# syun88/VLA-from-FastVLM

Measured on AMD Instinct MI355X. Metric: policy steps/sec (img+prompt->action) FastVLM-0.5B bs=64, higher is better.
Workload: dtype bf16; 1 GPU; fastvlm-0.5b select_action: letterbox 336^2->1024^2, FastViT-HD, projector, Qwen2 decoder (text-only, reference-literal: 64-token prompt), last-token pool, action head; batch_per_gpu=64, global_batch=64, seq_len=64, image=336, parallelism=replicas x1 (no collective on the inference path), tower_microbatch=0, stream_overlap=True, llm_precision=split-bf16 (hi+lo) operands, fp32 attention

## Files before the change

vla-from-fastvlm_amd/csrc/tower_kernels.hip:

```cpp
#include "kernels.h"
#include <cstdlib>

namespace fv {
namespace {

struct LbParams {
  const void* img; bf16_t* pix; int dtype, B, C, Hin, Win, S, rh, rw, pt, pl; float pad, sh, sw;
};

__device__ __forceinline__ float lb_fetch(const LbParams& p, size_t plane, int y, int x) {
  const size_t i = plane + (size_t)y * p.Win + x;
  return p.dtype == FV_U8 ? (float)static_cast<const uint8_t*>(p.img)[i] : static_cast<const float*>(p.img)[i];
}

__device__ __forceinline__ float lb_lerp(float a, float b, float w) {
#pragma clang fp contract(off)
  return (1.0f - w) * a + w * b;
}
__device__ __forceinline__ float lb_src(int d, float scale) {
#pragma clang fp contract(off)
  return fmaxf(((float)d + 0.5f) * scale - 0.5f, 0.0f);
}
__device__ __forceinline__ float lb_frac(float s, int i) {
#pragma clang fp contract(off)
// ... 497 lines not shown
        *reinterpret_cast<uint4*>(y + (((size_t)b * S2 + oy) * S2 + ox) * SF_C + cg * 8) = o;
      }
    }
    if (tile_n < (unsigned)ntiles) patch_store();
  }
}

typedef __attribute__((ext_vector_type(4))) short s16x4;

template <int K, int TH>
__global__ __launch_bounds__(256, TH == 8 ? 3 : 2) void dwconv_mfma_kernel(const bf16_t* __restrict__ x, const bf16_t* __restrict__ ttab,
                                                              const float* __restrict__ bias, bf16_t* __restrict__ y,
                                                              int H, int W, int C, int gelu, int tiles_x, int tiles_y,
                                                              int nslices) {
  constexpr int TW = 32, NP = TH / 8, PAD = K / 2, IH = TH + K - 1, IW = TW + K - 1;
  constexpr int NQ = (IW + 3) / 4, NM = (K + 3 + 3) / 4;
  constexpr int RS = NQ * 256 + 64;
  constexpr int T_BYTES = 2 * K * NM * 512, X_BYTES = IH * RS;
  __shared__ __attribute__((aligned(16))) char smem[X_BYTES];
  char* sX = smem;

  const int tid = threadIdx.x, lane = tid & 63, wid = tid >> 6;
#ifdef DW_NO_XCD
  int bid = blockIdx.x;
#else
  int bid = xcd_remap(blockIdx.x, gridDim.x);
#endif
  const int slice = bid % nslices; bid /= nslices;
  const int tx = bid % tiles_x; bid /= tiles_x;
  const int tyb = bid % tiles_y;
  const long b = bid / tiles_y;
  const int c0 = slice * 32;
  const int gg = wid & 1, rg = wid >> 1;
  const int bch = lane >> 2, jr = lane & 3;

  s16x4 afr[K][NM];
  {
    const char* tsrc = reinterpret_cast<const char*>(ttab) + (size_t)slice * T_BYTES + (size_t)gg * K * NM * 512 + lane * 8;
#pragma unroll
    for (int ky = 0; ky < K; ++ky)
#pragma unroll
      for (int m = 0; m < NM; ++m) afr[ky][m] = __builtin_bit_cast(s16x4, *reinterpret_cast<const uint2*>(tsrc + (ky * NM + m) * 512));
  }
  constexpr int NTASK = IH * NQ * 4, TPT = (NTASK + 255) / 256;
  uint4 px[TPT][4];
#pragma unroll
  for (int tt = 0; tt < TPT; ++tt) {
    const int task = tid + 256 * tt;
    const int cg = task & 3, quad = (task >> 2) % NQ, row = (task >> 2) / NQ;
    const int iy = tyb * TH - PAD + row, ix0 = tx * TW - PAD + quad * 4;
#pragma unroll
    for (int j = 0; j < 4; ++j) {
      const int ix = ix0 + j;
      px[tt][j] = (task < NTASK && iy >= 0 && iy < H && ix >= 0 && ix < W && quad * 4 + j < IW)
                      ? *reinterpret_cast<const uint4*>(x + (((size_t)b * H + iy) * W + ix) * C + c0 + cg * 8)
                      : make_uint4(0, 0, 0, 0);
    }
  }
#pragma unroll
  for (int tt = 0; tt < TPT; ++tt) {
    const int task = tid + 256 * tt;
    if (task < NTASK) {
      const int cg = task & 3, quad = (task >> 2) % NQ, row = (task >> 2) / NQ;
      const uint32_t d[4][4] = {{px[tt][0].x, px[tt][0].y, px[tt][0].z, px[tt][0].w}, {px[tt][1].x, px[tt][1].y, px[tt][1].z, px[tt][1].w},
                                {px[tt][2].x, px[tt][2].y, px[tt][2].z, px[tt][2].w}, {px[tt][3].x, px[tt][3].y, px[tt][3].z, px[tt][3].w}};
      const uint32_t dst = (uint32_t)(row * RS + quad * 256 + cg * 64) | (uint32_t)((((quad & 3) << 1) | (cg >> 1)) << 3);
#pragma unroll
      for (int dd = 0; dd < 4; ++dd) {
        uint2 ev, od;
        ev.x = __builtin_amdgcn_perm(d[1][dd], d[0][dd], 0x05040100u);
        ev.y = __builtin_amdgcn_perm(d[3][dd], d[2][dd], 0x05040100u);
        od.x = __builtin_amdgcn_perm(d[1][dd], d[0][dd], 0x07060302u);
        od.y = __builtin_amdgcn_perm(d[3][dd], d[2][dd], 0x07060302u);
        *reinterpret_cast<uint2*>(sX + (dst ^ (uint32_t)((2 * dd) * 8))) = ev;
        *reinterpret_cast<uint2*>(sX + (dst ^ (uint32_t)((2 * dd + 1) * 8))) = od;
      }
    }
  }
  __syncthreads();

  const char* lrow[4];
#pragma unroll
  for (int v = 0; v < 4; ++v) lrow[v] = sX + (rg * 4 * NP + jr) * RS + (((gg * 16 + bch) ^ ((v << 1) | gg)) << 3);
  f32x4 acc[NP][8];
#pragma unroll
  for (int pp = 0; pp < NP; ++pp)
#pragma unroll
    for (int q = 0; q < 8; ++q) acc[pp][q] = f32x4{0.f, 0.f, 0.f, 0.f};
#pragma unroll
  for (int pp = 0; pp < NP; ++pp)
#pragma unroll
    for (int ky = 0; ky < K; ++ky) {
      s16x4 xq[NQ];
#pragma unroll
      for (int t = 0; t < NQ; ++t)
        xq[t] = __builtin_bit_cast(s16x4, *reinterpret_cast<const uint2*>(lrow[t & 3] + (pp * 4 + ky) * RS + t * 256));
#pragma unroll
      for (int q = 0; q < 8; ++q)
#pragma unroll
        for (int m = 0; m < NM; ++m)
#ifdef DW_ABL_MFMA
          if (q + m < NQ && m == 0) acc[pp][q] = __builtin_amdgcn_mfma_f32_4x4x4bf16_1k(afr[ky][m], xq[q + m], acc[pp][q], 0, 0, 0);
#else
          if (q + m < NQ) acc[pp][q] = __builtin_amdgcn_mfma_f32_4x4x4bf16_1k(afr[ky][m], xq[q + m], acc[pp][q], 0, 0, 0);
#endif
    }
  __syncthreads();

  {
    const float bv = bias[c0 + gg * 16 + bch];
#pragma unroll
    for (int pp = 0; pp < NP; ++pp)
#pragma unroll
      for (int q = 0; q < 8; ++q) {
        float v[4];
#pragma unroll
        for (int i = 0; i < 4; ++i) {
          v[i] = acc[pp][q][i] + bv;
          if (gelu) v[i] = gelu_f(v[i]);
        }
        uint2 u;
        u.x = pack_bf2(v[0], v[1]);
        u.y = pack_bf2(v[2], v[3]);
        *reinterpret_cast<uint2*>(const_cast<char*>(lrow[q & 3]) + pp * 4 * RS + q * 256) = u;
      }
  }
  __syncthreads();
#pragma unroll
  for (int ot = 0; ot < NP; ++ot) {
    const int task = tid + 256 * ot;
    const int cg = task & 3, quad = (task >> 2) & 7, row = task >> 5;
    const uint32_t src = (uint32_t)(row * RS + quad * 256 + cg * 64) | (uint32_t)((((quad & 3) << 1) | (cg >> 1)) << 3);
    uint2 r[8];
#pragma unroll
    for (int e = 0; e < 8; ++e) r[e] = *reinterpret_cast<const uint2*>(sX + (src ^ (uint32_t)(e * 8)));
    const int oy = tyb * TH + row, ox0 = tx * TW + quad * 4;
    if (oy < H) {
      bf16_t* yp = y + (((size_t)b * H + oy) * W + ox0) * C + c0 + cg * 8;
#pragma unroll
      for (int j = 0; j < 4; ++j) {
        if (ox0 + j < W) {
          uint4 o;
          const uint32_t sel = (j & 1) ? 0x07060302u : 0x05040100u;
#define FV_PX(A, B) __builtin_amdgcn_perm((j & 2) ? r[B].y : r[B].x, (j & 2) ? r[A].y : r[A].x, sel)
          o.x = FV_PX(0, 1); o.y = FV_PX(2, 3); o.z = FV_PX(4, 5); o.w = FV_PX(6, 7);
#undef FV_PX
          *reinterpret_cast<uint4*>(yp + (size_t)j * C) = o;
        }
      }
    }
  }
}

__global__ __launch_bounds__(256, 2) void dwconv_s2_mfma_kernel(const bf16_t* __restrict__ x, const bf16_t* __restrict__ ttab,
                                                                 const float* __restrict__ bias, bf16_t* __restrict__ y, int H,
                                                                 int W, int C, int Ho, int Wo, int gelu, int tiles_x, int tiles_y,
                                                                 int nslices, int nimg) {
  constexpr int K = 7, TH = 8, TW = 16, PAD = 3, IH = 2 * TH + K - 2, IW = 2 * TW + K - 2;
  constexpr int NQ = (IW + 3) / 4, NM = 4;
  constexpr int RS = NQ * 256 + 64;
  constexpr int X_BYTES = IH * RS;
  constexpr int OC = 512 + 16;
  static_assert(TH * 4 * OC <= X_BYTES, "the output tile reuses the halo tile's LDS");
  __shared__ __attribute__((aligned(16))) char smem[X_BYTES];
  char* sX = smem;
  const int tid = threadIdx.x, lane = tid & 63, wid = tid >> 6;
  const int xcd = blockIdx.x & 7, lb = blockIdx.x >> 3;
  const int slice = lb % nslices, chain = lb / nslices, chains = (int)(gridDim.x >> 3) / nslices;
  const int ntiles = nimg * tiles_x * tiles_y;
  const int tpx = (ntiles + 7) >> 3, t_end = min((xcd + 1) * tpx, ntiles), per_slice = chains;
  const int c0 = slice * 32;
  const int gg = wid & 1, eo = wid >> 1;
  const int bch = lane >> 2, jr = lane & 3;

  s16x4 afr[K][NM];
  {
    const char* tsrc = reinterpret_cast<const char*>(ttab) + (size_t)(slice * 2 + gg) * (2 * K * NM * 512) + (size_t)eo * (K * NM * 512) + lane * 8;
#pragma unroll
    for (int ky = 0; ky < K; ++ky)
#pragma unroll
      for (int m = 0; m < NM; ++m) afr[ky][m] = __builtin_bit_cast(s16x4, *reinterpret_cast<const uint2*>(tsrc + (ky * NM + m) * 512));
  }
  constexpr int NTASK = IH * NQ * 4, TPT = (NTASK + 255) / 256;
  uint4 px[TPT][4];
  int trow[TPT], tcol[TPT], toff[TPT];
  uint32_t tdst[TPT];
#pragma unroll
  for (int tt = 0; tt < TPT; ++tt) {
    const int task = min(tid + 256 * tt, NTASK - 1);
    const int cg = task & 3, quad = (task >> 2) % NQ, row = (task >> 2) / NQ;
    trow[tt] = row;
    tcol[tt] = quad * 4;
    toff[tt] = (row * W + quad * 4) * C + cg * 8;
    tdst[tt] = (uint32_t)(row * RS + quad * 256 + cg * 64) | (uint32_t)((((quad & 3) << 1) | (cg >> 1)) << 3);
  }
  auto fetch = [&](int tx, int tyb, int b) {
    const int iy0 = 2 * tyb * TH - PAD, ix0 = 2 * tx * TW - PAD;
    const bf16_t* org = x + ((long)b * H * W + (long)iy0 * W + ix0) * C + c0;
#pragma unroll
    for (int tt = 0; tt < TPT; ++tt) {
      const bool rok = (unsigned)(iy0 + trow[tt]) < (unsigned)H;
#pragma unroll
      for (int j = 0; j < 4; ++j)
        px[tt][j] = (rok && (unsigned)(ix0 + tcol[tt] + j) < (unsigned)W) ? *reinterpret_cast<const uint4*>(org + toff[tt] + j * C)
                                                                         : make_uint4(0, 0, 0, 0);
    }
  };
  auto decode = [&](int tile, int& tx, int& tyb, int& b) {
    const unsigned t = (unsigned)tile, r = t / (unsigned)tiles_x;
    tx = (int)(t - r * (unsigned)tiles_x);
    b = (int)(r / (unsigned)tiles_y);
    tyb = (int)(r - (unsigned)b * (unsigned)tiles_y);
  };
  int tile = xcd * tpx + chain, tx = 0, tyb = 0, b = 0, txn = 0, tybn = 0, bn = 0;
  if (tile < t_end) { decode(tile, tx, tyb, b); fetch(tx, tyb, b); }
  for (; tile < t_end; tile += per_slice) {
#pragma unroll
  for (int tt = 0; tt < TPT; ++tt) {
    if (tid + 256 * tt < NTASK) {
      const uint32_t d[4][4] = {{px[tt][0].x, px[tt][0].y, px[tt][0].z, px[tt][0].w}, {px[tt][1].x, px[tt][1].y, px[tt][1].z, px[tt][1].w},
                                {px[tt][2].x, px[tt][2].y, px[tt][2].z, px[tt][2].w}, {px[tt][3].x, px[tt][3].y, px[tt][3].z, px[tt][3].w}};
      const uint32_t dst = tdst[tt];
#pragma unroll
      for (int dd = 0; dd < 4; ++dd) {
        uint2 ev, od;
        ev.x = __builtin_amdgcn_perm(d[1][dd], d[0][dd], 0x05040100u);
        ev.y = __builtin_amdgcn_perm(d[3][dd], d[2][dd], 0x05040100u);
        od.x = __builtin_amdgcn_perm(d[1][dd], d[0][dd], 0x07060302u);
        od.y = __builtin_amdgcn_perm(d[3][dd], d[2][dd], 0x07060302u);
        *reinterpret_cast<uint2*>(sX + (dst ^ (uint32_t)((2 * dd) * 8))) = ev;
        *reinterpret_cast<uint2*>(sX + (dst ^ (uint32_t)((2 * dd + 1) * 8))) = od;
      }
    }
  }
  __syncthreads();
  if (tile + per_slice < t_end) { decode(tile + per_slice, txn, tybn, bn); fetch(txn, tybn, bn); }

  const char* lrow[4];
#pragma unroll
  for (int v = 0; v < 4; ++v) lrow[v] = sX + (2 * jr) * RS + (((gg * 16 + bch) ^ ((v << 1) | gg)) << 3);
  f32x4 acc[2][4];
#pragma unroll
  for (int rg = 0; rg < 2; ++rg)
#pragma unroll
    for (int q = 0; q < 4; ++q) acc[rg][q] = f32x4{0.f, 0.f, 0.f, 0.f};
#pragma unroll
  for (int ky = 0; ky < K; ++ky)
#pragma unroll
    for (int rg = 0; rg < 2; ++rg) {
      s16x4 xq[NQ];
#pragma unroll
      for (int t = 0; t < NQ; ++t) xq[t] = __builtin_bit_cast(s16x4, *reinterpret_cast<const uint2*>(lrow[t & 3] + (rg * 8 + ky) * RS + t * 256));
#pragma unroll
      for (int m = 0; m < NM; ++m)
#pragma unroll
        for (int q = 0; q < 4; ++q) acc[rg][q] = __builtin_amdgcn_mfma_f32_4x4x4bf16_1k(afr[ky][m], xq[2 * q + m], acc[rg][q], 0, 0, 0);
    }
  __syncthreads();

  {
    const int co = 2 * (gg * 16 + bch) + eo, sig = (jr >> 1) & 1;
    const float bv = bias[2 * c0 + co];
#pragma unroll
    for (int rg = 0; rg < 2; ++rg)
#pragma unroll
      for (int q = 0; q < 4; ++q) {
        f32x2 g[2] = {{acc[rg][q][0] + bv, acc[rg][q][1] + bv}, {acc[rg][q][2] + bv, acc[rg][q][3] + bv}};
        if (gelu) gelu2_n<2>(g);
        uint2 u;
        u.x = pack_bf2(g[0].x, g[0].y);
        u.y = pack_bf2(g[1].x, g[1].y);
        *reinterpret_cast<uint2*>(sX + ((rg * 4 + jr) * 4 + q) * OC + ((co ^ sig) << 3)) = u;
      }
  }
  __syncthreads();
  {
    const int cg = tid & 7, quad = (tid >> 3) & 3, row = tid >> 5;
    const int sig = (row >> 1) & 1;
    uint2 r[8];
#pragma unroll
    for (int e = 0; e < 8; ++e) r[e] = *reinterpret_cast<const uint2*>(sX + (row * 4 + quad) * OC + (((cg * 8 + e) ^ sig) << 3));
    const int oy = tyb * TH + row, ox0 = tx * TW + quad * 4;
    if (oy < Ho) {
      bf16_t* yp = y + (((size_t)b * Ho + oy) * Wo + ox0) * (2 * C) + 2 * c0 + cg * 8;
#pragma unroll
      for (int j = 0; j < 4; ++j) {
        if (ox0 + j < Wo) {
          uint4 o;
          const uint32_t sel = (j & 1) ? 0x07060302u : 0x05040100u;
#define FV_PX(A, B) __builtin_amdgcn_perm((j & 2) ? r[B].y : r[B].x, (j & 2) ? r[A].y : r[A].x, sel)
          o.x = FV_PX(0, 1); o.y = FV_PX(2, 3); o.z = FV_PX(4, 5); o.w = FV_PX(6, 7);
#undef FV_PX
          *reinterpret_cast<uint4*>(yp + (size_t)j * (2 * C)) = o;
        }
      }
    }
  }
  __syncthreads();
  tx = txn; tyb = tybn; b = bn;
  }
}

#ifndef DW_MARCH_OCC
#define DW_MARCH_OCC 2
#endif
typedef __attribute__((ext_vector_type(4))) _Float16 f16x4_t;
template <int K, bool GRAD = false>
__global__ __launch_bounds__(256, DW_MARCH_OCC) void dwconv_march_kernel(const bf16_t* __restrict__ x, const bf16_t* __restrict__ ttab,
                                                               const float* __restrict__ bias, bf16_t* __restrict__ y,
                                                               int H, int W, int C, int gelu, int tiles_x, int nslices, const bf16_t* __restrict__ res = nullptr) {
  constexpr int TW = 32, PAD = K / 2, IW = TW + K - 1;
  constexpr int NQ = (IW + 3) / 4, NM = (K + 3 + 3) / 4;
  constexpr int RS = NQ * 256 + 64, RSO = 8 * 256 + 64;
  constexpr int T_BYTES = 2 * K * NM * 512;
#if DW_MARCH_OCC >= 3
  __shared__ __attribute__((aligned(16))) char smem[16 * RS];
#else
  __shared__ __attribute__((aligned(16))) char smem[16 * RS + 8 * RSO];
#endif
  char* sX = smem;

  const int tid = threadIdx.x, lane = tid & 63, wid = tid >> 6;
  int bid = xcd_remap(blockIdx.x, gridDim.x);
  const int slice = bid % nslices; bid /= nslices;
  const int tx = bid % tiles_x;
  const long b = bid / tiles_x;
  const int c0 = slice * 32;
  const int gg = wid & 1, rg = wid >> 1;
  const int bch = lane >> 2, jr = lane & 3;
  const int ng = (H + 7) / 8;

  s16x4 afr[K][NM];
  {
    const char* tsrc = reinterpret_cast<const char*>(ttab) + (size_t)slice * T_BYTES + (size_t)gg * K * NM * 512 + lane * 8;
#pragma unroll
    for (int ky = 0; ky < K; ++ky)
#pragma unroll
      for (int m = 0; m < NM; ++m) afr[ky][m] = __builtin_bit_cast(s16x4, *reinterpret_cast<const uint2*>(tsrc + (ky * NM + m) * 512));
  }
  const float bv = GRAD ? 0.f : bias[c0 + gg * 16 + bch];

  constexpr int NTASK = 8 * NQ * 4, TPT = (NTASK + 255) / 256;
  uint4 px[TPT][4];
#define DW_LOAD_UNIT(U)                                                                                          \
  {                                                                                                              \
    _Pragma("unroll") for (int tt = 0; tt < TPT; ++tt) {                                                         \
      const int task = tid + 256 * tt;                                                                           \
      const int cg = task & 3, quad = (task >> 2) % NQ, row = (task >> 2) / NQ;                                  \
      const int iy = 8 * (U) + PAD + row, ix0 = tx * TW - PAD + quad * 4;                                        \
      _Pragma("unroll") for (int j = 0; j < 4; ++j) {                                                            \
        const int ix = ix0 + j;                                                                                  \
        px[tt][j] = (task < NTASK && iy >= 0 && iy < H && ix >= 0 && ix < W && quad * 4 + j < IW)                \
                        ? *reinterpret_cast<const uint4*>(x + (((size_t)b * H + iy) * W + ix) * C + c0 + cg * 8)  \
                        : make_uint4(0, 0, 0, 0);                                                                \
      }                                                                                                          \
    }                                                                                                            \
  }
#define DW_WRITE_UNIT(U)                                                                                         \
  {                                                                                                              \
    _Pragma("unroll") for (int tt = 0; tt < TPT; ++tt) {                                                         \
      const int task = tid + 256 * tt;                                                                           \
      if (task < NTASK) {                                                                                        \
        const int cg = task & 3, quad = (task >> 2) % NQ, row = (task >> 2) / NQ;                                \
        const uint32_t d[4][4] = {{px[tt][0].x, px[tt][0].y, px[tt][0].z, px[tt][0].w},                          \
                                  {px[tt][1].x, px[tt][1].y, px[tt][1].z, px[tt][1].w},                          \
                                  {px[tt][2].x, px[tt][2].y, px[tt][2].z, px[tt][2].w},                          \
                                  {px[tt][3].x, px[tt][3].y, px[tt][3].z, px[tt][3].w}};                         \
        const uint32_t dst = (uint32_t)((8 * ((U) & 1) + row) * RS + quad * 256 + cg * 64) |                     \
                             (uint32_t)((((quad & 3) << 1) | (cg >> 1)) << 3);                                   \
        _Pragma("unroll") for (int dd = 0; dd < 4; ++dd) {                                                       \
          uint2 ev, od;                                                                                          \
          ev.x = __builtin_amdgcn_perm(d[1][dd], d[0][dd], 0x05040100u);                                         \
          ev.y = __builtin_amdgcn_perm(d[3][dd], d[2][dd], 0x05040100u);                                         \
          od.x = __builtin_amdgcn_perm(d[1][dd], d[0][dd], 0x07060302u);                                         \
          od.y = __builtin_amdgcn_perm(d[3][dd], d[2][dd], 0x07060302u);                                         \
          *reinterpret_cast<uint2*>(sX + (dst ^ (uint32_t)((2 * dd) * 8))) = ev;                                 \
          *reinterpret_cast<uint2*>(sX + (dst ^ (uint32_t)((2 * dd + 1) * 8))) = od;                             \
        }                                                                                                        \
      }                                                                                                          \
    }                                                                                                            \
  }
  uint32_t sw[4];
#pragma unroll
  for (int v = 0; v < 4; ++v) sw[v] = (uint32_t)(((gg * 16 + bch) ^ ((v << 1) | gg)) << 3);

  DW_LOAD_UNIT(-1)
  DW_WRITE_UNIT(-1)
  DW_LOAD_UNIT(0)
  DW_WRITE_UNIT(0)
  if (ng > 1) DW_LOAD_UNIT(1)

  for (int g = 0; g < ng; ++g) {
    __syncthreads();
    f32x4 acc[8];
#pragma unroll
    for (int q = 0; q < 8; ++q) acc[q] = f32x4{0.f, 0.f, 0.f, 0.f};
    const int rb = 8 * g + rg * 4 + jr - 2 * PAD;
#pragma unroll
    for (int ky = 0; ky < K; ++ky) {
      const uint32_t ro = (uint32_t)((rb + ky) & 15) * RS;
      s16x4 xq[NQ];
#pragma unroll
      for (int t = 0; t < NQ; ++t) xq[t] = __builtin_bit_cast(s16x4, *reinterpret_cast<const uint2*>(sX + ro + sw[t & 3] + t * 256));
#pragma unroll
      for (int m = 0; m < NM; ++m)
#pragma unroll
        for (int q = 0; q < 8; ++q)
          if (q + m < NQ) {
            if constexpr (GRAD) acc[q] = __builtin_amdgcn_mfma_f32_4x4x4f16(__builtin_bit_cast(f16x4_t, afr[ky][m]), __builtin_bit_cast(f16x4_t, xq[q + m]), acc[q], 0, 0, 0);
            else acc[q] = __builtin_amdgcn_mfma_f32_4x4x4bf16_1k(afr[ky][m], xq[q + m], acc[q], 0, 0, 0);
          }
    }
    __syncthreads();
#if DW_MARCH_OCC >= 3
    char* sO = sX + 8 * ((g + 1) & 1) * RS;
#else
    char* sO = smem + 16 * RS;
    if (g + 1 < ng) DW_WRITE_UNIT(g + 1)
    if (g + 2 < ng) DW_LOAD_UNIT(g + 2)
#endif
    {
      char* orow = sO + (rg * 4 + jr) * RSO;
#pragma unroll
      for (int q = 0; q < 8; ++q) {
        float v[4];
#pragma unroll
        for (int i = 0; i < 4; ++i) {
          v[i] = acc[q][i] + bv;
          if (gelu) v[i] = gelu_f(v[i]);
        }
        uint2 u;
        if constexpr (GRAD) { u.x = pack_h2(v[0], v[1]); u.y = pack_h2(v[2], v[3]); }
        else { u.x = pack_bf2(v[0], v[1]); u.y = pack_bf2(v[2], v[3]); }
        *reinterpret_cast<uint2*>(orow + sw[q & 3] + q * 256) = u;
      }
    }
    __syncthreads();
    {
      const int cg = tid & 3, quad = (tid >> 2) & 7, row = tid >> 5;
      const uint32_t src = (uint32_t)(row * RSO + quad * 256 + cg * 64) | (uint32_t)((((quad & 3) << 1) | (cg >> 1)) << 3);
      uint2 r[8];
#pragma unroll
      for (int e = 0; e < 8; ++e) r[e] = *reinterpret_cast<const uint2*>(sO + (src ^ (uint32_t)(e * 8)));
      const int oy = g * 8 + row, ox0 = tx * TW + quad * 4;
      if (oy < H) {
        bf16_t* yp = y + (((size_t)b * H + oy) * W + ox0) * C + c0 + cg * 8;
#pragma unroll
        for (int j = 0; j < 4; ++j) {
          if (ox0 + j < W) {
            uint4 o;
            const uint32_t sel = (j & 1) ? 0x07060302u : 0x05040100u;
#define FV_PX(A, B) __builtin_amdgcn_perm((j & 2) ? r[B].y : r[B].x, (j & 2) ? r[A].y : r[A].x, sel)
// ... 489 lines not shown
  p.img = img; p.pix = pix; p.dtype = dtype; p.B = B; p.C = C; p.Hin = Hin; p.Win = Win; p.S = S; p.pad = pad_value;
  if (letterbox) {
    const double ratio = ((double)Win / S > (double)Hin / S) ? (double)Win / S : (double)Hin / S;
    p.rh = (int)((double)Hin / ratio);
    p.rw = (int)((double)Win / ratio);
    if (p.rh > S || p.rw > S || p.rh < 1 || p.rw < 1) return fv_fail(FV_ERR_ARG, "letterbox: degenerate resize %dx%d", p.rh, p.rw);
  } else {
    p.rh = S; p.rw = S;
  }
  p.pt = S - p.rh; p.pl = S - p.rw;
  p.sh = (float)Hin / (float)p.rh;
  p.sw = (float)Win / (float)p.rw;
  return FV_OK;
}
}

int launch_letterbox(const void* img, int dtype, int B, int C, int Hin, int Win, int S, float pad_value, int letterbox,
                     bf16_t* pix, hipStream_t s) {
  if (!img || !pix) return fv_fail(FV_ERR_ARG, "letterbox: null pointer");
  LbParams p;
  FV_TRY_RC(lb_params(img, dtype, B, C, Hin, Win, S, pad_value, letterbox, pix, p));
  hipLaunchKernelGGL(letterbox_kernel<0>, dim3((S + 255) / 256, (S + LB_R - 1) / LB_R, B), dim3(256), 0, s, p, LbNorm{});
  FV_HIP_CHECK(hipGetLastError());
  return FV_OK;
}

int launch_letterbox_norm(const void* img, int dtype, int B, int C, int Hin, int Win, int S, float pad_value, int letterbox, const float* mean3,
                          const float* std3, int range_heuristic, unsigned* vmax_scratch, bf16_t* pix, hipStream_t s) {
  if (!img || !pix || !mean3 || !std3 || (range_heuristic && !vmax_scratch)) return fv_fail(FV_ERR_ARG, "letterbox_norm: null pointer");
  LbParams p;
  FV_TRY_RC(lb_params(img, dtype, B, C, Hin, Win, S, pad_value, letterbox, pix, p));
  LbNorm n{};
  for (int c = 0; c < 3; ++c) {
    if (!(std3[c] != 0.0f)) return fv_fail(FV_ERR_ARG, "letterbox_norm: std[%d] must be non-zero", c);
    n.mean[c] = mean3[c]; n.std[c] = std3[c];
  }
  n.vmax = vmax_scratch; n.heuristic = range_heuristic ? 1 : 0;
  const dim3 grid((S + 255) / 256, (S + LB_R - 1) / LB_R, B);
  if (range_heuristic) {
    FV_HIP_CHECK(hipMemsetAsync(vmax_scratch, 0, 4, s));
    hipLaunchKernelGGL(letterbox_kernel<1>, grid, dim3(256), 0, s, p, n);
  }
  hipLaunchKernelGGL(letterbox_kernel<2>, grid, dim3(256), 0, s, p, n);
  FV_HIP_CHECK(hipGetLastError());
  return FV_OK;
}

int launch_stem_conv(const bf16_t* pix, const float* w, const float* bias, bf16_t* y, int B, int S, int Cout,
                     hipStream_t s) {
  if (!pix || !w || !bias || !y) return fv_fail(FV_ERR_ARG, "stem_conv: null pointer");
  if (B <= 0 || S < 2 || (S & 1) || Cout % 8 || Cout < 8 || Cout > 2048) return fv_fail(FV_ERR_ARG, "stem_conv: bad shape S=%d Cout=%d", S, Cout);
  const int So = S / 2, G = Cout / 8, WQ = (So + 3) / 4, per_block = 256 / G;
  const long quads = (long)B * So * WQ;
  const long blocks = (quads + per_block - 1) / per_block;
  hipLaunchKernelGGL(stem_conv_kernel, dim3((unsigned)blocks), dim3(256), 27 * Cout * sizeof(float), s, pix, w, bias, y, B, S, Cout);
  FV_HIP_CHECK(hipGetLastError());
  return FV_OK;
}

void stem_mfma_pack(const float* w27, float* out, int Cout) {
  for (int co = 0; co < Cout; ++co)
    for (int ks = 0; ks < 2; ++ks)
      for (int g = 0; g < 4; ++g)
        for (int e = 0; e < 8; ++e) {
          const int ky = 2 * ks + (g >> 1), kx = 2 * (g & 1) + (e >> 2), ch = e & 3;
          out[(size_t)co * 64 + ks * 32 + g * 8 + e] = (ky < 3 && kx < 3 && ch < 3) ? w27[(size_t)((ky * 3 + kx) * 3 + ch) * Cout + co] : 0.0f;
        }
}

int launch_stem_mfma(const bf16_t* pix, const bf16_t* wp, const float* bias, bf16_t* y, int B, int S, int Cout, hipStream_t s) {
  if (!pix || !wp || !bias || !y) return fv_fail(FV_ERR_ARG, "stem_mfma: null pointer");
  if (B <= 0 || S < 2 || (S & 1) || Cout % 16 || Cout > 128) return fv_fail(FV_ERR_UNSUPPORTED, "stem_mfma: bad shape S=%d Cout=%d", S, Cout);
  const int So = S / 2;
  const long ntiles = (long)B * So * ((So + 15) / 16);
  constexpr int TPW = 8;
  const long blocks = (ntiles + 4 * TPW - 1) / (4 * TPW);
  hipLaunchKernelGGL(stem_mfma_kernel<TPW>, dim3((unsigned)blocks), dim3(256), 0, s, pix, wp, bias, y, B, S, Cout, ntiles);
  FV_HIP_CHECK(hipGetLastError());
  return FV_OK;
}

int launch_dwconv(const bf16_t* x, const float* w, const float* bias, bf16_t* y, int B, int H, int W, int C, int k,
                  int stride, int mult, int gelu, hipStream_t s) {
  if (!x || !w || !bias || !y) return fv_fail(FV_ERR_ARG, "dwconv: null pointer");
  if (B <= 0 || H <= 0 || W <= 0 || C <= 0 || (C * mult) % 8) return fv_fail(FV_ERR_ARG, "dwconv: bad shape C=%d mult=%d", C, mult);
  const int pad = k / 2;
  const int Ho = (H + 2 * pad - k) / stride + 1, Wo = (W + 2 * pad - k) / stride + 1;
  if (stride == 1 && mult == 1 && (k == 3 || k == 7) && W >= 32 && C % 32 == 0) {
    const int tiles_x = (W + 31) / 32, tiles_y = (H + 7) / 8, nsl = C / 32;
    const long nblk = (long)B * tiles_x * tiles_y * nsl;
    if (nblk > 0x7fffffffL) return fv_fail(FV_ERR_ARG, "dwconv: grid too large");
    if (k == 7) hipLaunchKernelGGL(dwconv_tile_kernel<7>, dim3((unsigned)nblk), dim3(256), 0, s, x, w, bias, y, H, W, C, gelu, tiles_x, tiles_y, nsl);
    else hipLaunchKernelGGL(dwconv_tile_kernel<3>, dim3((unsigned)nblk), dim3(256), 0, s, x, w, bias, y, H, W, C, gelu, tiles_x, tiles_y, nsl);
    FV_HIP_CHECK(hipGetLastError());
    return FV_OK;
  }
  const int G = C * mult / 8, WQ = (Wo + 3) / 4;
  int GS = 1;
  for (int d = 1; d <= 16; ++d)
    if (G % d == 0) GS = d;
  const int nslices = G / GS, qpb = 256 / GS;
  const long nquads = (long)B * Ho * WQ;
  const long blocks = (nquads + qpb - 1) / qpb * nslices;
  if (blocks > 0x7fffffffL) return fv_fail(FV_ERR_ARG, "dwconv: grid too large");
  const dim3 grid((unsigned)blocks);
#define FV_DW(K_, S_, M_)                                                                                        \
  if (k == K_ && stride == S_ && mult == M_) {                                                                   \
    hipLaunchKernelGGL((dwconv_kernel<K_, S_, M_>), grid, dim3(256), 0, s, x, w, bias, y, B, H, W, C, Ho, Wo, gelu, \
                       GS, nslices, nquads);                                                                     \
    FV_HIP_CHECK(hipGetLastError());                                                                             \
    return FV_OK;                                                                                                \
  }
  FV_DW(3, 1, 1) FV_DW(7, 1, 1) FV_DW(3, 2, 1) FV_DW(7, 2, 2) FV_DW(3, 1, 2)
#undef FV_DW
  return fv_fail(FV_ERR_UNSUPPORTED, "dwconv: unsupported k=%d stride=%d mult=%d", k, stride, mult);
}

size_t dwconv_toeplitz_elems(int C, int k) { return (size_t)(C / 16) * k * ((k + 6) / 4) * 256; }
void dwconv_toeplitz_pack(const float* w_tapmajor, float* out, int C, int k) {
  const int NM = (k + 6) / 4;
  for (int g = 0; g < C / 16; ++g)
    for (int ky = 0; ky < k; ++ky)
      for (int m = 0; m < NM; ++m)
        for (int bch = 0; bch < 16; ++bch)
          for (int i = 0; i < 4; ++i)
            for (int kk = 0; kk < 4; ++kk) {
              const int kx = 4 * m + kk - i;
              out[((((size_t)(g * k + ky) * NM + m) * 16 + bch) * 4 + i) * 4 + kk] =
                  (kx >= 0 && kx < k) ? w_tapmajor[(size_t)(ky * k + kx) * C + g * 16 + bch] : 0.0f;
            }
}
size_t dwconv_s2_toeplitz_elems(int C) { return (size_t)(C / 16) * 2 * 7 * 4 * 256; }
void dwconv_s2_toeplitz_pack(const float* w_tapmajor, float* out, int C) {
  for (int g = 0; g < C / 16; ++g)
    for (int e = 0; e < 2; ++e)
      for (int ky = 0; ky < 7; ++ky)
        for (int m = 0; m < 4; ++m)
          for (int bch = 0; bch < 16; ++bch)
            for (int i = 0; i < 4; ++i)
              for (int kk = 0; kk < 4; ++kk) {
                const int kx = 4 * m + kk - 2 * i;
                out[(((((size_t)(g * 2 + e) * 7 + ky) * 4 + m) * 16 + bch) * 4 + i) * 4 + kk] =
                    (kx >= 0 && kx < 7) ? w_tapmajor[(size_t)(ky * 7 + kx) * (2 * C) + 2 * (g * 16 + bch) + e] : 0.0f;
              }
}
bool dwconv_s2_mfma_supported(int H, int W, int C, int k, int stride, int mult) {
  return k == 7 && stride == 2 && mult == 2 && C % 32 == 0 && H % 2 == 0 && W % 2 == 0 && W >= 16;
}
int launch_dwconv_s2_mfma(const bf16_t* x, const bf16_t* ttab, const float* bias, bf16_t* y, int B, int H, int W, int C, int gelu,
                          hipStream_t s) {
  if (!x || !ttab || !bias || !y) return fv_fail(FV_ERR_ARG, "dwconv_s2_mfma: null pointer");
  if (B <= 0 || H <= 0 || !dwconv_s2_mfma_supported(H, W, C, 7, 2, 2)) return fv_fail(FV_ERR_UNSUPPORTED, "dwconv_s2_mfma: unsupported shape H=%d W=%d C=%d", H, W, C);
  const int Ho = H / 2, Wo = W / 2;
  const int tiles_x = (Wo + 15) / 16, tiles_y = (Ho + 7) / 8, nsl = C / 32;
  const long nblk = (long)B * tiles_x * tiles_y * nsl;
  if (nblk > 0x7fffffffL) return fv_fail(FV_ERR_ARG, "dwconv_s2_mfma: grid too large");
  static int cus = 0;
  if (!cus) {
    int dev = 0;
    hipDeviceProp_t prop;
    cus = (hipGetDevice(&dev) == hipSuccess && hipGetDeviceProperties(&prop, dev) == hipSuccess && prop.multiProcessorCount > 0) ? prop.multiProcessorCount : 256;
  }
  const long tiles = nblk / nsl, tpx = (tiles + 7) / 8;
  long chains = (2L * cus / 8) / nsl;
  if (chains < 1) chains = 1;
  if (chains > tpx) chains = tpx;
  hipLaunchKernelGGL(dwconv_s2_mfma_kernel, dim3((unsigned)(8 * chains * nsl)), dim3(256), 0, s, x, ttab, bias, y, H, W, C, Ho, Wo, gelu, tiles_x, tiles_y, nsl, B);
  FV_HIP_CHECK(hipGetLastError());
  return FV_OK;
}

bool dwconv_mfma_supported(int W, int C, int k, int stride, int mult) {
  return stride == 1 && mult == 1 && (k == 3 || k == 7) && W >= 16 && C % 32 == 0;
}

int launch_dwconv_mfma(const bf16_t* x, const bf16_t* ttab, const float* bias, bf16_t* y, int B, int H, int W, int C, int k,
                       int gelu, hipStream_t s) {
  if (!x || !ttab || !bias || !y) return fv_fail(FV_ERR_ARG, "dwconv_mfma: null pointer");
  if (B <= 0 || H <= 0 || !dwconv_mfma_supported(W, C, k, 1, 1)) return fv_fail(FV_ERR_UNSUPPORTED, "dwconv_mfma: unsupported shape W=%d C=%d k=%d", W, C, k);
#ifndef DW_TH7
#define DW_TH7 8
#endif
  const int th = (k == 7 && H >= 32) ? DW_TH7 : 8;
  const int tiles_x = (W + 31) / 32, tiles_y = (H + th - 1) / th, nsl = C / 32;
  const long nblk = (long)B * tiles_x * tiles_y * nsl;
  if (nblk > 0x7fffffffL) return fv_fail(FV_ERR_ARG, "dwconv_mfma: grid too large");
#ifndef DW_NO_MARCH
  if (k == 7 && H >= 16) {
    const long nstrips = (long)B * tiles_x * nsl;
    hipLaunchKernelGGL((dwconv_march_kernel<7>), dim3((unsigned)nstrips), dim3(256), 0, s, x, ttab, bias, y, H, W, C, gelu, tiles_x, nsl);
    FV_HIP_CHECK(hipGetLastError());
    return FV_OK;
  }
#ifdef DW_MARCH3
  if (k == 3 && H >= 16) {
    const long nstrips = (long)B * tiles_x * nsl;
    hipLaunchKernelGGL((dwconv_march_kernel<3>), dim3((unsigned)nstrips), dim3(256), 0, s, x, ttab, bias, y, H, W, C, gelu, tiles_x, nsl);
    FV_HIP_CHECK(hipGetLastError());
    return FV_OK;
  }
#endif
#endif
  if (k == 7 && th == 16) hipLaunchKernelGGL((dwconv_mfma_kernel<7, 16>), dim3((unsigned)nblk), dim3(256), 0, s, x, ttab, bias, y, H, W, C, gelu, tiles_x, tiles_y, nsl);
  else if (k == 7) hipLaunchKernelGGL((dwconv_mfma_kernel<7, 8>), dim3((unsigned)nblk), dim3(256), 0, s, x, ttab, bias, y, H, W, C, gelu, tiles_x, tiles_y, nsl);
  else hipLaunchKernelGGL((dwconv_mfma_kernel<3, 8>), dim3((unsigned)nblk), dim3(256), 0, s, x, ttab, bias, y, H, W, C, gelu, tiles_x, tiles_y, nsl);
  FV_HIP_CHECK(hipGetLastError());
  return FV_OK;
}

bool dw_dgrad_mfma_supported(int H, int W, int C, int k) { return dwconv_mfma_supported(W, C, k, 1, 1) && H >= 16; }
int launch_dw_dgrad_mfma(const bf16_t* dy, const bf16_t* ttab16, const bf16_t* res, bf16_t* dx, int B, int H, int W, int C, int k, hipStream_t s) {
  if (!dy || !ttab16 || !dx) return fv_fail(FV_ERR_ARG, "dw_dgrad_mfma: null pointer");
  if (B <= 0 || !dw_dgrad_mfma_supported(H, W, C, k)) return fv_fail(FV_ERR_UNSUPPORTED, "dw_dgrad_mfma: unsupported shape H=%d W=%d C=%d k=%d", H, W, C, k);
  const int tiles_x = (W + 31) / 32, nsl = C / 32;
  const long nstrips = (long)B * tiles_x * nsl;
  if (nstrips > 0x7fffffffL) return fv_fail(FV_ERR_ARG, "dw_dgrad_mfma: grid too large");
  if (k == 7) hipLaunchKernelGGL((dwconv_march_kernel<7, true>), dim3((unsigned)nstrips), dim3(256), 0, s, dy, ttab16, static_cast<const float*>(nullptr), dx, H, W, C, 0, tiles_x, nsl, res);
  else hipLaunchKernelGGL((dwconv_march_kernel<3, true>), dim3((unsigned)nstrips), dim3(256), 0, s, dy, ttab16, static_cast<const float*>(nullptr), dx, H, W, C, 0, tiles_x, nsl, res);
  FV_HIP_CHECK(hipGetLastError());
  return FV_OK;
}

bool stem_fused_supported(int S, int C0) { return C0 == SF_C && S >= 8 && S % 4 == 0; }
int launch_stem_fused(const bf16_t* pix, const bf16_t* wp, const float* b1, const float* w2, const float* b2, bf16_t* y, int B,
                      int S, int C0, hipStream_t s) {
  if (!pix || !wp || !b1 || !w2 || !b2 || !y) return fv_fail(FV_ERR_ARG, "stem_fused: null pointer");
  if (B <= 0 || !stem_fused_supported(S, C0)) return fv_fail(FV_ERR_UNSUPPORTED, "stem_fused: bad shape S=%d C0=%d", S, C0);
  static bool attr_set = false;
  if (!attr_set) {
    FV_HIP_CHECK(hipFuncSetAttribute(reinterpret_cast<const void*>(&stem_fused_kernel<false>), hipFuncAttributeMaxDynamicSharedMemorySize, SF_LDS));
    attr_set = true;
  }
  const int S2 = S / 4;
  const long ntiles = (long)B * ((S2 + SF_TC - 1) / SF_TC) * ((S2 + SF_TR - 1) / SF_TR);
  if (ntiles > 0x3fffffffL) return fv_fail(FV_ERR_ARG, "stem_fused: too many tiles");
  int dev = 0, cus = 256;
  hipDeviceProp_t prop;
  if (hipGetDevice(&dev) == hipSuccess && hipGetDeviceProperties(&prop, dev) == hipSuccess && prop.multiProcessorCount > 0) cus = prop.multiProcessorCount;
  const long blocks = ntiles < cus ? ntiles : cus;
  hipLaunchKernelGGL(stem_fused_kernel<false>, dim3((unsigned)blocks), dim3(512), SF_LDS, s, pix, wp, b1, w2, b2, y, B, S, ntiles, LbParams{});
  FV_HIP_CHECK(hipGetLastError());
  return FV_OK;
}

int launch_stem_fused_lb(const void* img, int dtype, int B, int C, int Hin, int Win, float pad_value, int letterbox, const bf16_t* wp,
                         const float* b1, const float* w2, const float* b2, bf16_t* y, int S, int C0, hipStream_t s) {
  if (!img || !wp || !b1 || !w2 || !b2 || !y) return fv_fail(FV_ERR_ARG, "stem_fused_lb: null pointer");
  if (B <= 0 || !stem_fused_supported(S, C0)) return fv_fail(FV_ERR_UNSUPPORTED, "stem_fused_lb: bad shape S=%d C0=%d", S, C0);
  LbParams p;
  FV_TRY_RC(lb_params(img, dtype, B, C, Hin, Win, S, pad_value, letterbox, nullptr, p));
  static bool attr_set = false;
  if (!attr_set) {
    FV_HIP_CHECK(hipFuncSetAttribute(reinterpret_cast<const void*>(&stem_fused_kernel<true>), hipFuncAttributeMaxDynamicSharedMemorySize, SF_LDS));
    attr_set = true;
  }
  const int S2 = S / 4;
  const long ntiles = (long)B * ((S2 + SF_TC - 1) / SF_TC) * ((S2 + SF_TR - 1) / SF_TR);
  if (ntiles > 0x3fffffffL) return fv_fail(FV_ERR_ARG, "stem_fused_lb: too many tiles");
  int dev = 0, cus = 256;
  hipDeviceProp_t prop;
  if (hipGetDevice(&dev) == hipSuccess && hipGetDeviceProperties(&prop, dev) == hipSuccess && prop.multiProcessorCount > 0) cus = prop.multiProcessorCount;
  const long blocks = ntiles < cus ? ntiles : cus;
  hipLaunchKernelGGL(stem_fused_kernel<true>, dim3((unsigned)blocks), dim3(512), SF_LDS, s, nullptr, wp, b1, w2, b2, y, B, S, ntiles, p);
  FV_HIP_CHECK(hipGetLastError());
  return FV_OK;
}

bool dwconv_pair_supported(int B, int H, int W, int C) {
  return H >= 16 && W >= 32 && C % 32 == 0 && ((long)B * H + 16) * W * C * 2 <= 0x7FFFFFF0L;
}
int launch_dwconv_pair(const bf16_t* x, const bf16_t* t3, const float* b3, const bf16_t* t7, const float* b7, bf16_t* y1, bf16_t* y2,
                       int B, int H, int W, int C, hipStream_t s) {
  if (!x || !t3 || !b3 || !t7 || !b7 || !y1 || !y2) return fv_fail(FV_ERR_ARG, "dwconv_pair: null pointer");
  if (B <= 0 || !dwconv_pair_supported(B, H, W, C)) return fv_fail(FV_ERR_UNSUPPORTED, "dwconv_pair: unsupported shape H=%d W=%d C=%d", H, W, C);
  if (x == y1 || x == y2 || y1 == y2) return fv_fail(FV_ERR_ARG, "dwconv_pair: buffers must be distinct");
  static bool attr_set = false;
  if (!attr_set) {
    FV_HIP_CHECK(hipFuncSetAttribute(reinterpret_cast<const void*>(&dwpair_march_kernel<32, 32>), hipFuncAttributeMaxDynamicSharedMemorySize, DpGeo<32, 32>::LDS));
    FV_HIP_CHECK(hipFuncSetAttribute(reinterpret_cast<const void*>(&dwpair_march_kernel<64, 16>), hipFuncAttributeMaxDynamicSharedMemorySize, DpGeo<64, 16>::LDS));
    FV_HIP_CHECK(hipFuncSetAttribute(reinterpret_cast<const void*>(&dwpair_march_kernel<32, 16>), hipFuncAttributeMaxDynamicSharedMemorySize, DpGeo<32, 16>::LDS));
#if DP_DEFAULT_GEO == 3
    FV_HIP_CHECK(hipFuncSetAttribute(reinterpret_cast<const void*>(&dwpair_march_kernel<64, 8>), hipFuncAttributeMaxDynamicSharedMemorySize, DpGeo<64, 8>::LDS));
#endif
    attr_set = true;
  }
  int geo = DP_DEFAULT_GEO;
  if ((geo == 1 || geo == 3) && C % 64) geo = 0;
  const int chb = (geo == 1 || geo == 3) ? 64 : 32, tw = geo == 0 ? 32 : geo == 3 ? 8 : 16;
  const int tiles_x = (W + tw - 1) / tw, nsl = C / chb;
  long nstrips = (long)B * tiles_x * nsl;
  if (nstrips > 0x7fffffffL) return fv_fail(FV_ERR_ARG, "dwconv_pair: grid too large");
  int nseg = 1;
  if (nstrips < 256) {
    const int ng = (H + 7) / 8;
    nseg = (int)((512 + nstrips - 1) / nstrips);
    if (nseg > ng / 2) nseg = ng / 2;
    if (nseg < 1) nseg = 1;
  }
  nstrips *= nseg;
#if DP_DEFAULT_GEO == 3
  if (geo == 3)
    hipLaunchKernelGGL((dwpair_march_kernel<64, 8>), dim3((unsigned)nstrips), dim3(256), (DpGeo<64, 8>::LDS), s, x, t3, b3, t7, b7, y1, y2, H, W, C, tiles_x, nsl, nseg);
  else
#endif
  if (geo == 1)
    hipLaunchKernelGGL((dwpair_march_kernel<64, 16>), dim3((unsigned)nstrips), dim3(256), (DpGeo<64, 16>::LDS), s, x, t3, b3, t7, b7, y1, y2, H, W, C, tiles_x, nsl, nseg);
  else if (geo == 2)
    hipLaunchKernelGGL((dwpair_march_kernel<32, 16>), dim3((unsigned)nstrips), dim3(256), (DpGeo<32, 16>::LDS), s, x, t3, b3, t7, b7, y1, y2, H, W, C, tiles_x, nsl, nseg);
  else
    hipLaunchKernelGGL((dwpair_march_kernel<32, 32>), dim3((unsigned)nstrips), dim3(256), (DpGeo<32, 32>::LDS), s, x, t3, b3, t7, b7, y1, y2, H, W, C, tiles_x, nsl, nseg);
  FV_HIP_CHECK(hipGetLastError());
  return FV_OK;
}

int launch_layernorm_rows(const bf16_t* x, const float* w, const float* b, bf16_t* y, int rows, int C, float eps,
                          hipStream_t s) {
  if (!x || !w || !b || !y) return fv_fail(FV_ERR_ARG, "layernorm_rows: null pointer");
  if (rows <= 0 || C % 8 || C > 2048 || C <= 0) return fv_fail(FV_ERR_ARG, "layernorm_rows: bad shape rows=%d C=%d", rows, C);
  hipLaunchKernelGGL(layernorm_rows_kernel, dim3((rows + 3) / 4), dim3(256), 0, s, x, w, b, y, rows, C, eps);
  FV_HIP_CHECK(hipGetLastError());
// ... 25 lines not shown
```

Measured before the change: 19.15 steps/s.

## Restructure stride-2 dwconv as vertical marching ring buffer with channel slabs

The stride-2 7x7 depthwise MFMA kernel no longer uses persistent chains over independent 8x16 tiles. Each block now marches down a column segment and keeps a 16-row ring buffer of halo rows in LDS, so each step loads only the new input rows, and the next rows are prefetched while the current ones are computed. Channel slabs are templated at 32, 64 or 96 channels with block sizes to match, and the launcher splits columns into segments to fill the CUs. The intent is to stop re-reading the vertical halo rows that overlapping tiles shared, at the cost of more dynamic LDS, lower occupancy and extra code paths.

Result: no change. 19.29 steps/s (median of 6 runs) (+0.7%).

```diff
diff --git a/vla-from-fastvlm_amd/csrc/tower_kernels.hip b/vla-from-fastvlm_amd/csrc/tower_kernels.hip
--- a/vla-from-fastvlm_amd/csrc/tower_kernels.hip
+++ b/vla-from-fastvlm_amd/csrc/tower_kernels.hip
@@ -673,51 +673,67 @@
   }
 }
 
-__global__ __launch_bounds__(256, 2) void dwconv_s2_mfma_kernel(const bf16_t* __restrict__ x, const bf16_t* __restrict__ ttab,
+template <int CHB>
+struct S2Geo {
+  static constexpr int TW = 16, NQ = 10, NPL = CHB / 32, PLB = NQ * 256, RS = NPL * PLB + 16;
+  static constexpr int NT = CHB * 8;
+  static constexpr int NCG = CHB / 8;
+  static constexpr int NCGO = CHB / 4;
+  static constexpr int OC = 2 * CHB * 9 + 16;
+  static constexpr int RING = 16 * RS, LDS = RING + 16 * OC;
+  static constexpr int WPE = CHB == 64 ? 2 : 3;
+};
+template <int CHB>
+__global__ __launch_bounds__(S2Geo<CHB>::NT, S2Geo<CHB>::WPE) void dwconv_s2_mfma_kernel(const bf16_t* __restrict__ x, const bf16_t* __restrict__ ttab,
                                                                  const float* __restrict__ bias, bf16_t* __restrict__ y, int H,
-                                                                 int W, int C, int Ho, int Wo, int gelu, int tiles_x, int tiles_y,
-                                                                 int nslices, int nimg) {
-  constexpr int K = 7, TH = 8, TW = 16, PAD = 3, IH = 2 * TH + K - 2, IW = 2 * TW + K - 2;
-  constexpr int NQ = (IW + 3) / 4, NM = 4;
-  constexpr int RS = NQ * 256 + 64;
-  constexpr int X_BYTES = IH * RS;
-  constexpr int OC = 512 + 16;
-  static_assert(TH * 4 * OC <= X_BYTES, "the output tile reuses the halo tile's LDS");
-  __shared__ __attribute__((aligned(16))) char smem[X_BYTES];
-  char* sX = smem;
+                                                                 int W, int C, int Ho, int Wo, int gelu, int tiles_x, int nslab, int nseg) {
+  using G = S2Geo<CHB>;
+  constexpr int K = 7, NM = 4, NQ = G::NQ, RS = G::RS, PLB = G::PLB, OC = G::OC, NT = G::NT, NCG = G::NCG, NCGO = G::NCGO;
+  extern __shared__ __attribute__((aligned(16))) char s2_smem[];
+  char* sX = s2_smem;
+  char* sO = s2_smem + G::RING;
   const int tid = threadIdx.x, lane = tid & 63, wid = tid >> 6;
-  const int xcd = blockIdx.x & 7, lb = blockIdx.x >> 3;
-  const int slice = lb % nslices, chain = lb / nslices, chains = (int)(gridDim.x >> 3) / nslices;
-  const int ntiles = nimg * tiles_x * tiles_y;
-  const int tpx = (ntiles + 7) >> 3, t_end = min((xcd + 1) * tpx, ntiles), per_slice = chains;
-  const int c0 = slice * 32;
-  const int gg = wid & 1, eo = wid >> 1;
+  int bid = xcd_remap(blockIdx.x, gridDim.x);
+  const int slab = bid % nslab; bid /= nslab;
+  const int seg = bid % nseg; bid /= nseg;
+  const int tx = bid % tiles_x;
+  const long b = bid / tiles_x;
+  const int c0 = slab * CHB;
+  const int gg = wid >> 1, eo = wid & 1;
   const int bch = lane >> 2, jr = lane & 3;
+  const int ng = (Ho + 3) >> 2;
+  const int g0 = (int)((long)seg * ng / nseg), g1 = (int)((long)(seg + 1) * ng / nseg);
 
   s16x4 afr[K][NM];
   {
-    const char* tsrc = reinterpret_cast<const char*>(ttab) + (size_t)(slice * 2 + gg) * (2 * K * NM * 512) + (size_t)eo * (K * NM * 512) + lane * 8;
+    const char* tsrc = reinterpret_cast<const char*>(ttab) + (size_t)((c0 >> 4) + gg) * (2 * K * NM * 512) + (size_t)eo * (K * NM * 512) + lane * 8;
 #pragma unroll
     for (int ky = 0; ky < K; ++ky)
 #pragma unroll
       for (int m = 0; m < NM; ++m) afr[ky][m] = __builtin_bit_cast(s16x4, *reinterpret_cast<const uint2*>(tsrc + (ky * NM + m) * 512));
   }
-  constexpr int NTASK = IH * NQ * 4, TPT = (NTASK + 255) / 256;
+  const int co = 2 * (gg * 16 + bch) + eo;
+  const float bv = bias[2 * c0 + co];
+
+  constexpr int NTASK = 8 * NQ * NCG, TPT = (NTASK + NT - 1) / NT;
   uint4 px[TPT][4];
   int trow[TPT], tcol[TPT], toff[TPT];
-  uint32_t tdst[TPT];
+  uint32_t tdst[TPT], tsw[TPT];
 #pragma unroll
   for (int tt = 0; tt < TPT; ++tt) {
-    const int task = min(tid + 256 * tt, NTASK - 1);
-    const int cg = task & 3, quad = (task >> 2) % NQ, row = (task >> 2) / NQ;
-    trow[tt] = row;
+    const int task = min(tid + NT * tt, NTASK - 1);
+    const int cg = task % NCG, quad = (task / NCG) % NQ, row = task / (NCG * NQ);
+    trow[tt] = tid + NT * tt < NTASK ? row : -0x40000000;
     tcol[tt] = quad * 4;
     toff[tt] = (row * W + quad * 4) * C + cg * 8;
-    tdst[tt] = (uint32_t)(row * RS + quad * 256 + cg * 64) | (uint32_t)((((quad & 3) << 1) | (cg >> 1)) << 3);
-  }
-  auto fetch = [&](int tx, int tyb, int b) {
-    const int iy0 = 2 * tyb * TH - PAD, ix0 = 2 * tx * TW - PAD;
-    const bf16_t* org = x + ((long)b * H * W + (long)iy0 * W + ix0) * C + c0;
+    tdst[tt] = (uint32_t)(row * RS + (cg >> 2) * PLB + quad * 256 + (cg & 3) * 64);
+    tsw[tt] = (uint32_t)((((quad * G::NPL + (cg >> 2)) & 3) << 1) | ((cg & 3) >> 1));
+  }
+  const int ix0 = 2 * tx * G::TW - 3;
+  const bf16_t* xim = x + (long)b * H * W * C + c0;
+  auto fetch = [&](int u) {
+    const int iy0 = 8 * u + 2;
+    const bf16_t* org = xim + ((long)iy0 * W + ix0) * C;
 #pragma unroll
     for (int tt = 0; tt < TPT; ++tt) {
       const bool rok = (unsigned)(iy0 + trow[tt]) < (unsigned)H;
@@ -727,98 +743,96 @@
                                                                          : make_uint4(0, 0, 0, 0);
     }
   };
-  auto decode = [&](int tile, int& tx, int& tyb, int& b) {
-    const unsigned t = (unsigned)tile, r = t / (unsigned)tiles_x;
-    tx = (int)(t - r * (unsigned)tiles_x);
-    b = (int)(r / (unsigned)tiles_y);
-    tyb = (int)(r - (unsigned)b * (unsigned)tiles_y);
+  auto stash = [&](int u) {
+    char* ring = sX + 8 * (u & 1) * RS;
+#pragma unroll
+    for (int tt = 0; tt < TPT; ++tt) {
+      if (tid + NT * tt < NTASK) {
+        const uint32_t d[4][4] = {{px[tt][0].x, px[tt][0].y, px[tt][0].z, px[tt][0].w}, {px[tt][1].x, px[tt][1].y, px[tt][1].z, px[tt][1].w},
+                                  {px[tt][2].x, px[tt][2].y, px[tt][2].z, px[tt][2].w}, {px[tt][3].x, px[tt][3].y, px[tt][3].z, px[tt][3].w}};
+#pragma unroll
+        for (int dd = 0; dd < 4; ++dd) {
+          uint2 ev, od;
+          ev.x = __builtin_amdgcn_perm(d[1][dd], d[0][dd], 0x05040100u);
+          ev.y = __builtin_amdgcn_perm(d[3][dd], d[2][dd], 0x05040100u);
+          od.x = __builtin_amdgcn_perm(d[1][dd], d[0][dd], 0x07060302u);
+          od.y = __builtin_amdgcn_perm(d[3][dd], d[2][dd], 0x07060302u);
+          *reinterpret_cast<uint2*>(ring + tdst[tt] + ((tsw[tt] ^ (uint32_t)(2 * dd)) << 3)) = ev;
+          *reinterpret_cast<uint2*>(ring + tdst[tt] + ((tsw[tt] ^ (uint32_t)(2 * dd + 1)) << 3)) = od;
+        }
+      }
+    }
   };
-  int tile = xcd * tpx + chain, tx = 0, tyb = 0, b = 0, txn = 0, tybn = 0, bn = 0;
-  if (tile < t_end) { decode(tile, tx, tyb, b); fetch(tx, tyb, b); }
-  for (; tile < t_end; tile += per_slice) {
-#pragma unroll
-  for (int tt = 0; tt < TPT; ++tt) {
-    if (tid + 256 * tt < NTASK) {
-      const uint32_t d[4][4] = {{px[tt][0].x, px[tt][0].y, px[tt][0].z, px[tt][0].w}, {px[tt][1].x, px[tt][1].y, px[tt][1].z, px[tt][1].w},
-                                {px[tt][2].x, px[tt][2].y, px[tt][2].z, px[tt][2].w}, {px[tt][3].x, px[tt][3].y, px[tt][3].z, px[tt][3].w}};
-      const uint32_t dst = tdst[tt];
-#pragma unroll
-      for (int dd = 0; dd < 4; ++dd) {
-        uint2 ev, od;
-        ev.x = __builtin_amdgcn_perm(d[1][dd], d[0][dd], 0x05040100u);
-        ev.y = __builtin_amdgcn_perm(d[3][dd], d[2][dd], 0x05040100u);
-        od.x = __builtin_amdgcn_perm(d[1][dd], d[0][dd], 0x07060302u);
-        od.y = __builtin_amdgcn_perm(d[3][dd], d[2][dd], 0x07060302u);
-        *reinterpret_cast<uint2*>(sX + (dst ^ (uint32_t)((2 * dd) * 8))) = ev;
-        *reinterpret_cast<uint2*>(sX + (dst ^ (uint32_t)((2 * dd + 1) * 8))) = od;
-      }
-    }
-  }
-  __syncthreads();
-  if (tile + per_slice < t_end) { decode(tile + per_slice, txn, tybn, bn); fetch(txn, tybn, bn); }
-
-  const char* lrow[4];
-#pragma unroll
-  for (int v = 0; v < 4; ++v) lrow[v] = sX + (2 * jr) * RS + (((gg * 16 + bch) ^ ((v << 1) | gg)) << 3);
-  f32x4 acc[2][4];
-#pragma unroll
-  for (int rg = 0; rg < 2; ++rg)
-#pragma unroll
-    for (int q = 0; q < 4; ++q) acc[rg][q] = f32x4{0.f, 0.f, 0.f, 0.f};
-#pragma unroll
-  for (int ky = 0; ky < K; ++ky)
-#pragma unroll
-    for (int rg = 0; rg < 2; ++rg) {
+  uint32_t sw[4];
+#pragma unroll
+  for (int v = 0; v < 4; ++v)
+    sw[v] = (uint32_t)((gg >> 1) * PLB) + (uint32_t)((((gg & 1) * 16 + bch) ^ ((((v * G::NPL + (gg >> 1)) & 3) << 1) | (gg & 1))) << 3);
+  const int sig = (jr >> 1) & 1;
+  const uint32_t oslot = (uint32_t)(co ^ sig);
+  char* const owr = sO + (jr * 4) * OC + ((oslot + (oslot >> 3)) << 3);
+  const int ocg = tid % NCGO, orest = tid / NCGO;
+  const int ohalf = orest & 1, oquad = (orest >> 1) & 3, orow = orest >> 3;
+  const int osig = (orow >> 1) & 1;
+  const char* const ord = sO + (orow * 4 + oquad) * OC + ocg * 72 + ohalf * 4;
+  const int ox0 = tx * G::TW + oquad * 4 + ohalf * 2;
+  bf16_t* const yim = y + (long)b * Ho * Wo * (2 * C) + 2 * c0 + ocg * 8;
+
+  fetch(g0 - 1);
+  stash(g0 - 1);
+  fetch(g0);
+  stash(g0);
+  if (g0 + 1 < g1) fetch(g0 + 1);
+
+  for (int g = g0; g < g1; ++g) {
+    __syncthreads();
+    f32x4 acc[4];
+#pragma unroll
+    for (int q = 0; q < 4; ++q) acc[q] = f32x4{0.f, 0.f, 0.f, 0.f};
+    const int rb = 8 * g + 2 * jr - 5;
+#pragma unroll
+    for (int ky = 0; ky < K; ++ky) {
+      const char* rrow = sX + (uint32_t)((rb + ky) & 15) * RS;
       s16x4 xq[NQ];
 #pragma unroll
-      for (int t = 0; t < NQ; ++t) xq[t] = __builtin_bit_cast(s16x4, *reinterpret_cast<const uint2*>(lrow[t & 3] + (rg * 8 + ky) * RS + t * 256));
+      for (int t = 0; t < NQ; ++t) xq[t] = __builtin_bit_cast(s16x4, *reinterpret_cast<const uint2*>(rrow + sw[t & 3] + t * 256));
 #pragma unroll
       for (int m = 0; m < NM; ++m)
 #pragma unroll
-        for (int q = 0; q < 4; ++q) acc[rg][q] = __builtin_amdgcn_mfma_f32_4x4x4bf16_1k(afr[ky][m], xq[2 * q + m], acc[rg][q], 0, 0, 0);
-    }
-  __syncthreads();
-
-  {
-    const int co = 2 * (gg * 16 + bch) + eo, sig = (jr >> 1) & 1;
-    const float bv = bias[2 * c0 + co];
-#pragma unroll
-    for (int rg = 0; rg < 2; ++rg)
-#pragma unroll
-      for (int q = 0; q < 4; ++q) {
-        f32x2 g[2] = {{acc[rg][q][0] + bv, acc[rg][q][1] + bv}, {acc[rg][q][2] + bv, acc[rg][q][3] + bv}};
-        if (gelu) gelu2_n<2>(g);
-        uint2 u;
-        u.x = pack_bf2(g[0].x, g[0].y);
-        u.y = pack_bf2(g[1].x, g[1].y);
-        *reinterpret_cast<uint2*>(sX + ((rg * 4 + jr) * 4 + q) * OC + ((co ^ sig) << 3)) = u;
-      }
-  }
-  __syncthreads();
-  {
-    const int cg = tid & 7, quad = (tid >> 3) & 3, row = tid >> 5;
-    const int sig = (row >> 1) & 1;
-    uint2 r[8];
-#pragma unroll
-    for (int e = 0; e < 8; ++e) r[e] = *reinterpret_cast<const uint2*>(sX + (row * 4 + quad) * OC + (((cg * 8 + e) ^ sig) << 3));
-    const int oy = tyb * TH + row, ox0 = tx * TW + quad * 4;
-    if (oy < Ho) {
-      bf16_t* yp = y + (((size_t)b * Ho + oy) * Wo + ox0) * (2 * C) + 2 * c0 + cg * 8;
-#pragma unroll
-      for (int j = 0; j < 4; ++j) {
-        if (ox0 + j < Wo) {
-          uint4 o;
-          const uint32_t sel = (j & 1) ? 0x07060302u : 0x05040100u;
-#define FV_PX(A, B) __builtin_amdgcn_perm((j & 2) ? r[B].y : r[B].x, (j & 2) ? r[A].y : r[A].x, sel)
-          o.x = FV_PX(0, 1); o.y = FV_PX(2, 3); o.z = FV_PX(4, 5); o.w = FV_PX(6, 7);
-#undef FV_PX
-          *reinterpret_cast<uint4*>(yp + (size_t)j * (2 * C)) = o;
+        for (int q = 0; q < 4; ++q) acc[q] = __builtin_amdgcn_mfma_f32_4x4x4bf16_1k(afr[ky][m], xq[2 * q + m], acc[q], 0, 0, 0);
+    }
+#pragma unroll
+    for (int q = 0; q < 4; ++q) {
+      f32x2 gv[2] = {{acc[q][0] + bv, acc[q][1] + bv}, {acc[q][2] + bv, acc[q][3] + bv}};
+      if (gelu) gelu2_n<2>(gv);
+      uint2 u;
+      u.x = pack_bf2(gv[0].x, gv[0].y);
+      u.y = pack_bf2(gv[1].x, gv[1].y);
+      *reinterpret_cast<uint2*>(owr + q * OC) = u;
+    }
+    __syncthreads();
+    if (g + 1 < g1) stash(g + 1);
+    if (g + 2 < g1) fetch(g + 2);
+    {
+      uint32_t r[8];
+#pragma unroll
+      for (int e = 0; e < 8; ++e) r[e] = *reinterpret_cast<const uint32_t*>(ord + ((e ^ osig) << 3));
+      const int oy = g * 4 + orow;
+      if (oy < Ho) {
+        bf16_t* yp = yim + ((long)oy * Wo + ox0) * (2 * C);
+#pragma unroll
+        for (int j = 0; j < 2; ++j) {
+          if (ox0 + j < Wo) {
+            const uint32_t sel = j ? 0x07060302u : 0x05040100u;
+            uint4 o;
+            o.x = __builtin_amdgcn_perm(r[1], r[0], sel);
+            o.y = __builtin_amdgcn_perm(r[3], r[2], sel);
+            o.z = __builtin_amdgcn_perm(r[5], r[4], sel);
+            o.w = __builtin_amdgcn_perm(r[7], r[6], sel);
+            *reinterpret_cast<uint4*>(yp + (long)j * (2 * C)) = o;
+          }
         }
       }
     }
-  }
-  __syncthreads();
-  tx = txn; tyb = tybn; b = bn;
   }
 }
 
@@ -1614,20 +1628,33 @@
   if (!x || !ttab || !bias || !y) return fv_fail(FV_ERR_ARG, "dwconv_s2_mfma: null pointer");
   if (B <= 0 || H <= 0 || !dwconv_s2_mfma_supported(H, W, C, 7, 2, 2)) return fv_fail(FV_ERR_UNSUPPORTED, "dwconv_s2_mfma: unsupported shape H=%d W=%d C=%d", H, W, C);
   const int Ho = H / 2, Wo = W / 2;
-  const int tiles_x = (Wo + 15) / 16, tiles_y = (Ho + 7) / 8, nsl = C / 32;
-  const long nblk = (long)B * tiles_x * tiles_y * nsl;
-  if (nblk > 0x7fffffffL) return fv_fail(FV_ERR_ARG, "dwconv_s2_mfma: grid too large");
+  const int chb = C % 64 == 0 ? 64 : C == 96 ? 96 : 32;
+  const int tiles_x = (Wo + 15) / 16, nslab = C / chb, ng = (Ho + 3) / 4;
+  long nblk = (long)B * tiles_x * nslab;
   static int cus = 0;
   if (!cus) {
     int dev = 0;
     hipDeviceProp_t prop;
     cus = (hipGetDevice(&dev) == hipSuccess && hipGetDeviceProperties(&prop, dev) == hipSuccess && prop.multiProcessorCount > 0) ? prop.multiProcessorCount : 256;
-  }
-  const long tiles = nblk / nsl, tpx = (tiles + 7) / 8;
-  long chains = (2L * cus / 8) / nsl;
-  if (chains < 1) chains = 1;
-  if (chains > tpx) chains = tpx;
-  hipLaunchKernelGGL(dwconv_s2_mfma_kernel, dim3((unsigned)(8 * chains * nsl)), dim3(256), 0, s, x, ttab, bias, y, H, W, C, Ho, Wo, gelu, tiles_x, tiles_y, nsl, B);
+    FV_HIP_CHECK(hipFuncSetAttribute(reinterpret_cast<const void*>(&dwconv_s2_mfma_kernel<32>), hipFuncAttributeMaxDynamicSharedMemorySize, S2Geo<32>::LDS));
+    FV_HIP_CHECK(hipFuncSetAttribute(reinterpret_cast<const void*>(&dwconv_s2_mfma_kernel<64>), hipFuncAttributeMaxDynamicSharedMemorySize, S2Geo<64>::LDS));
+    FV_HIP_CHECK(hipFuncSetAttribute(reinterpret_cast<const void*>(&dwconv_s2_mfma_kernel<96>), hipFuncAttributeMaxDynamicSharedMemorySize, S2Geo<96>::LDS));
+  }
+  int nseg = 1;
+  const long want = (long)cus * (chb == 32 ? 3 : 1);
+  if (nblk < want) {
+    nseg = (int)((want + nblk - 1) / nblk);
+    if (nseg > ng / 2) nseg = ng / 2;
+    if (nseg < 1) nseg = 1;
+  }
+  nblk *= nseg;
+  if (nblk > 0x7fffffffL) return fv_fail(FV_ERR_ARG, "dwconv_s2_mfma: grid too large");
+  if (chb == 64)
+    hipLaunchKernelGGL((dwconv_s2_mfma_kernel<64>), dim3((unsigned)nblk), dim3(S2Geo<64>::NT), S2Geo<64>::LDS, s, x, ttab, bias, y, H, W, C, Ho, Wo, gelu, tiles_x, nslab, nseg);
+  else if (chb == 96)
+    hipLaunchKernelGGL((dwconv_s2_mfma_kernel<96>), dim3((unsigned)nblk), dim3(S2Geo<96>::NT), S2Geo<96>::LDS, s, x, ttab, bias, y, H, W, C, Ho, Wo, gelu, tiles_x, nslab, nseg);
+  else
+    hipLaunchKernelGGL((dwconv_s2_mfma_kernel<32>), dim3((unsigned)nblk), dim3(S2Geo<32>::NT), S2Geo<32>::LDS, s, x, ttab, bias, y, H, W, C, Ho, Wo, gelu, tiles_x, nslab, nseg);
   FV_HIP_CHECK(hipGetLastError());
   return FV_OK;
 }
```
